# ueda0319/neddf

Measured on AMD Instinct MI355X. Metric: rendered rays/sec (800x800, 128 samples/ray), higher is better.
Workload: dtype f32

## Files before the change

### neddf_amd/csrc/tile_engine.h

```cpp
#pragma once
#include "kernels.h"
#include "device_math.h"

namespace neddf {

typedef float f32x16 __attribute__((ext_vector_type(16)));
typedef float f32x4v __attribute__((ext_vector_type(4)));
typedef __bf16 bf16x8 __attribute__((ext_vector_type(8)));
typedef unsigned short u16x4 __attribute__((ext_vector_type(4)));
typedef unsigned int u32x4 __attribute__((ext_vector_type(4)));

#ifdef NEDDF_EXACT_ACT
#define NEDDF_ACT_F32 0
#define NEDDF_ACT_SPLIT 0
#endif
#ifndef NEDDF_ACT_F32
#define NEDDF_ACT_F32 2
#endif
#ifndef NEDDF_ACT_SPLIT
#define NEDDF_ACT_SPLIT 2
#endif

template <int WID>
struct OpsF32T {
    static constexpr int kWid = WID;
    typedef float act_t;
    typedef f32x4v frag;
    typedef frag afrag;
    typedef frag bfrag;
    static constexpr int kLd = WID + 4;
    static constexpr int kStep = 8;
    static constexpr int kSub = 4;
    static constexpr bool kFast = false;
    static constexpr int kActMode = NEDDF_ACT_F32;
    static constexpr int kPlanes = 1, kPlane = 0;
    static constexpr bool kPackedRows = false;
    static constexpr float kWScale = 1.0f;
    static constexpr bool kStash16 = false;
    static constexpr bool kDeepPrefetch = false;
    static constexpr bool kEncInLds = false;
    static constexpr bool kTransposed = false, kStashF16 = false;
    typedef frag mfrag;
    static __device__ __forceinline__ frag load_a(const act_t *p) { return *(const frag *)p; }
    static __device__ __forceinline__ const mfrag &prep(const frag &a) { return a; }
    static __device__ __forceinline__ void zero(act_t *p) { *p = 0.f; }
    static __device__ __forceinline__ void put4(act_t *p, const f32x4v &v) { *(f32x4v *)p = v; }
    static __device__ __forceinline__ void put(act_t *p, float v) { *p = v; }
    static __device__ __forceinline__ void put2(act_t *pa, act_t *pb, float va, float vb) { *pa = va; *pb = vb; }
    static __device__ __forceinline__ float get(const act_t *p) { return *p; }
    static __device__ __forceinline__ void load4(const act_t *p, float (&x)[4])
    {
        f32x4v v = *(const f32x4v *)p;
        x[0] = v[0]; x[1] = v[1]; x[2] = v[2]; x[3] = v[3];
    }
    static __device__ __forceinline__ f32x16 mfma(const frag &a, const frag &b, const f32x16 &c, int r)
    {
        return __builtin_amdgcn_mfma_f32_32x32x2f32(a[r], b[r], c, 0, 0, 0);
    }
};

typedef OpsF32T<256> OpsF32;

template <int WID>
struct OpsBF16T {
    static constexpr int kWid = WID;
    typedef unsigned short act_t;
    typedef bf16x8 frag;
    typedef frag afrag;
    typedef frag bfrag;
    static constexpr int kLd = WID + 8;
    static constexpr int kStep = 16;
    static constexpr int kSub = 1;
    static constexpr bool kFast = true;
    static constexpr int kActMode = 1;
    static constexpr int kPlanes = 1, kPlane = 0;
    static constexpr float kWScale = 1.0f;
    static constexpr bool kStash16 = true;
    static constexpr bool kDeepPrefetch = true;
    static constexpr bool kEncInLds = true;
    static constexpr bool kTransposed = false, kStashF16 = false;
    typedef frag mfrag;
    static __device__ __forceinline__ frag load_a(const act_t *p) { return *(const frag *)p; }
    static __device__ __forceinline__ const mfrag &prep(const frag &a) { return a; }
    static __device__ __forceinline__ void zero(act_t *p) { *p = 0; }
    static __device__ __forceinline__ unsigned short cvt(float v)
    {
        typedef __bf16 bf16x2 __attribute__((ext_vector_type(2)));
        typedef float f32x2 __attribute__((ext_vector_type(2)));
        f32x2 in = { v, v };
        bf16x2 o = __builtin_convertvector(in, bf16x2);
        return __builtin_bit_cast(unsigned int, o) & 0xffffu;
    }
    static __device__ __forceinline__ void put(act_t *p, float v) { *p = cvt(v); }
    static __device__ __forceinline__ void put2(act_t *pa, act_t *pb, float va, float vb)
    {
        typedef __bf16 bf16x2 __attribute__((ext_vector_type(2)));
        typedef float f32x2 __attribute__((ext_vector_type(2)));
        const unsigned int w = __builtin_bit_cast(unsigned int, __builtin_convertvector((f32x2){ va, vb }, bf16x2));
        *pa = (unsigned short)w; *pb = (unsigned short)(w >> 16);
    }
    static constexpr bool kPackedRows = true;
    static __device__ __forceinline__ void put_rows4(act_t *p, int ld, float v0, float v1, float v2, float v3)
    {
        typedef __bf16 bf16x2 __attribute__((ext_vector_type(2)));
        typedef float f32x2 __attribute__((ext_vector_type(2)));
        const unsigned int a = __builtin_bit_cast(unsigned int, __builtin_convertvector((f32x2){ v0, v1 }, bf16x2));
        const unsigned int b = __builtin_bit_cast(unsigned int, __builtin_convertvector((f32x2){ v2, v3 }, bf16x2));
        p[0] = (unsigned short)a; p[ld] = (unsigned short)(a >> 16);
        p[2 * ld] = (unsigned short)b; p[3 * ld] = (unsigned short)(b >> 16);
    }
    static __device__ __forceinline__ float get(const act_t *p) { return __builtin_bit_cast(float, (unsigned int)*p << 16); }
    static __device__ __forceinline__ void load4(const act_t *p, float (&x)[4])
    {
        u16x4 v = *(const u16x4 *)p;
#pragma unroll
        for (int i = 0; i < 4; ++i) x[i] = __builtin_bit_cast(float, (unsigned int)v[i] << 16);
    }
    static __device__ __forceinline__ f32x16 mfma(const frag &a, const frag &b, const f32x16 &c, int)
    {
        return __builtin_amdgcn_mfma_f32_32x32x16_bf16(a, b, c, 0, 0, 0);
    }
};
typedef OpsBF16T<256> OpsBF16;

template <int WID>
struct OpsBF16RT : OpsBF16T<WID> {
    typedef OpsBF16T<WID> Base;
    typedef typename Base::act_t act_t;
    typedef typename Base::frag frag;
    static constexpr bool kTransposed = true, kStashF16 = true;
    static __device__ __forceinline__ f32x16 mfma(const frag &a, const frag &b, const f32x16 &c, int)
    {
        return __builtin_amdgcn_mfma_f32_32x32x16_bf16(b, a, c, 0, 0, 0);
    }
    static __device__ __forceinline__ void put4(act_t *p, float v0, float v1, float v2, float v3)
    {
        typedef __bf16 bf16x2 __attribute__((ext_vector_type(2)));
        typedef float f32x2 __attribute__((ext_vector_type(2)));
        typedef unsigned int u32x2 __attribute__((ext_vector_type(2)));
        u32x2 w = { __builtin_bit_cast(unsigned int, __builtin_convertvector((f32x2){ v0, v1 }, bf16x2)),
                    __builtin_bit_cast(unsigned int, __builtin_convertvector((f32x2){ v2, v3 }, bf16x2)) };
        *(u32x2 *)p = w;
    }
};

typedef _Float16 f16x8 __attribute__((ext_vector_type(8)));
struct hfrag2 {
    f16x8 h, m;
};

template <int WID>
struct OpsF16SplitT {
    static constexpr int kWid = WID;
    typedef unsigned short act_t;
    typedef hfrag2 afrag;
    typedef hfrag2 bfrag;
    static constexpr int kPlanes = 2, kPlane = WID + 8;
    static constexpr int kLd = 2 * (WID + 8) + 8;
    static constexpr int kStep = 16;
    static constexpr int kSub = 3;
    static constexpr bool kFast = false;
    static constexpr int kActMode = NEDDF_ACT_SPLIT;
    static constexpr bool kPackedRows = false;
    static constexpr float kWScale = 1024.0f;
    static constexpr bool kStash16 = false;
    static constexpr bool kDeepPrefetch = false;
    static constexpr bool kEncInLds = false;
    static constexpr bool kTransposed = false, kStashF16 = false;
    static __device__ __forceinline__ float f(unsigned short b) { return (float)__builtin_bit_cast(_Float16, b); }
    static __device__ __forceinline__ void put(act_t *p, float v)
    {
        typedef __fp16 h2 __attribute__((ext_vector_type(2)));
        h2 t = __builtin_amdgcn_cvt_pkrtz(v, v);
        const _Float16 h = (_Float16)t[0];
        const _Float16 m = (_Float16)__builtin_amdgcn_fmed3f(v - (float)h, -65504.0f, 65504.0f);
        p[0] = __builtin_bit_cast(unsigned short, h);
        p[kPlane] = __builtin_bit_cast(unsigned short, m);
    }
    static __device__ __forceinline__ void put2(act_t *pa, act_t *pb, float va, float vb) { put(pa, va); put(pb, vb); }
    static __device__ __forceinline__ void zero(act_t *p) { p[0] = 0; p[kPlane] = 0; }
    static __device__ __forceinline__ void put4(act_t *p, const f32x4v &v)
    {
        typedef __fp16 h2 __attribute__((ext_vector_type(2)));
        typedef _Float16 f16x4 __attribute__((ext_vector_type(4)));
        f16x4 h, m;
#pragma unroll
        for (int i = 0; i < 4; ++i) {
            h2 t = __builtin_amdgcn_cvt_pkrtz(v[i], v[i]);
            h[i] = (_Float16)t[0];
            m[i] = (_Float16)__builtin_amdgcn_fmed3f(v[i] - (float)h[i], -65504.0f, 65504.0f);
        }
        *(f16x4 *)p = h;
        *(f16x4 *)(p + kPlane) = m;
    }
    static __device__ __forceinline__ float get(const act_t *p) { return f(p[kPlane]) + f(p[0]); }
    static __device__ __forceinline__ void load4(const act_t *p, float (&x)[4])
    {
        u16x4 h = *(const u16x4 *)p, m = *(const u16x4 *)(p + kPlane);
#pragma unroll
        for (int i = 0; i < 4; ++i) x[i] = f(m[i]) + f(h[i]);
    }
    static __device__ __forceinline__ afrag load_a(const act_t *p)
    {
        afrag a;
        a.h = *(const f16x8 *)p; a.m = *(const f16x8 *)(p + kPlane);
        return a;
    }
    typedef afrag mfrag;
    static __device__ __forceinline__ const mfrag &prep(const afrag &a) { return a; }
    static __device__ __forceinline__ f32x16 mfma(const afrag &a, const bfrag &b, const f32x16 &c, int r)
    {
        switch (r) {
        case 0: return __builtin_amdgcn_mfma_f32_32x32x16_f16(a.m, b.h, c, 0, 0, 0);
        case 1: return __builtin_amdgcn_mfma_f32_32x32x16_f16(a.h, b.m, c, 0, 0, 0);
        default: return __builtin_amdgcn_mfma_f32_32x32x16_f16(a.h, b.h, c, 0, 0, 0);
        }
    }
};
typedef OpsF16SplitT<256> OpsF16Split;

struct f32x8frag {
    f32x4v lo, hi;
};
struct bf16x8x3 {
    bf16x8 t[3];
};

template <int WID>
struct OpsF32x3T : OpsF32T<WID> {
    typedef float act_t;
    typedef f32x8frag afrag;
    typedef bf16x8x3 bfrag;
    typedef bf16x8x3 mfrag;
    static constexpr int kStep = 16;
    static constexpr int kSub = 6;
    static __device__ __forceinline__ afrag load_a(const act_t *p) { return { *(const f32x4v *)p, *(const f32x4v *)(p + 4) }; }
    static __device__ __forceinline__ unsigned cvt2(float x0, float x1, float &y0, float &y1)
    {
        typedef __bf16 bf16x2 __attribute__((ext_vector_type(2)));
        typedef float f32x2 __attribute__((ext_vector_type(2)));
        unsigned w = __builtin_bit_cast(unsigned, __builtin_convertvector((f32x2){ x0, x1 }, bf16x2));
        asm("" : "+v"(w));
        y0 = __builtin_bit_cast(float, w << 16);
        y1 = __builtin_bit_cast(float, w & 0xffff0000u);
        return w;
    }
    static __device__ __forceinline__ mfrag prep(const afrag &a)
    {
        const float x[8] = { a.lo[0], a.lo[1], a.lo[2], a.lo[3], a.hi[0], a.hi[1], a.hi[2], a.hi[3] };
        u32x4 t0, t1, t2;
#pragma unroll
        for (int i = 0; i < 4; ++i) {
            float h0, h1, m0, m1, d0, d1;
            t0[i] = cvt2(x[2 * i], x[2 * i + 1], h0, h1);
            const float r0 = x[2 * i] - h0, r1 = x[2 * i + 1] - h1;
            t1[i] = cvt2(r0, r1, m0, m1);
            t2[i] = cvt2(r0 - m0, r1 - m1, d0, d1);
            (void)d0; (void)d1;
        }
        mfrag m;
        m.t[0] = __builtin_bit_cast(bf16x8, t0); m.t[1] = __builtin_bit_cast(bf16x8, t1); m.t[2] = __builtin_bit_cast(bf16x8, t2);
        return m;
    }
    static __device__ __forceinline__ f32x16 mfma(const mfrag &a, const bfrag &b, const f32x16 &c, int r)
    {
        switch (r) {
        case 0: return __builtin_amdgcn_mfma_f32_32x32x16_bf16(a.t[2], b.t[0], c, 0, 0, 0);
        case 1: return __builtin_amdgcn_mfma_f32_32x32x16_bf16(a.t[1], b.t[1], c, 0, 0, 0);
        case 2: return __builtin_amdgcn_mfma_f32_32x32x16_bf16(a.t[0], b.t[2], c, 0, 0, 0);
        case 3: return __builtin_amdgcn_mfma_f32_32x32x16_bf16(a.t[1], b.t[0], c, 0, 0, 0);
        case 4: return __builtin_amdgcn_mfma_f32_32x32x16_bf16(a.t[0], b.t[1], c, 0, 0, 0);
        default: return __builtin_amdgcn_mfma_f32_32x32x16_bf16(a.t[0], b.t[0], c, 0, 0, 0);
        }
    }
};

constexpr int kEncLd = 72;
template <class Ops>
struct EncView : Ops {
    static constexpr int kLd = kEncLd;
};

template <class Ops>
__device__ __forceinline__ const typename Ops::act_t *act_lane_ptr(const typename Ops::act_t *act, int lane)
{
    return act + (lane & 31) * Ops::kLd + (Ops::kStep / 2) * (lane >> 5);
}

struct WeightStream {
    __amdgpu_buffer_rsrc_t rsrc;
    unsigned lane_off;
};

template <class F>
__device__ __forceinline__ WeightStream weight_stream(const F *wl)
{
    const unsigned lane = __builtin_amdgcn_mbcnt_hi(~0u, __builtin_amdgcn_mbcnt_lo(~0u, 0u));
    const unsigned long long u = (unsigned long long)(wl - lane);
    const unsigned lo = __builtin_amdgcn_readfirstlane((unsigned)u), hi = __builtin_amdgcn_readfirstlane((unsigned)(u >> 32));
    void *base = (void *)(((unsigned long long)hi << 32) | lo);
    return { __builtin_amdgcn_make_buffer_rsrc(base, 0, (int)0xffffffffu, 0x00020000), lane * (unsigned)sizeof(F) };
}

template <class F>
__device__ __forceinline__ F stream_load(const WeightStream &w, unsigned frag_index)
{
    static_assert(sizeof(F) % 16 == 0, "fragments are fetched 16 bytes at a time");
    struct Raw { u32x4 v[sizeof(F) / 16]; } raw;
#pragma unroll
    for (unsigned i = 0; i < sizeof(F) / 16; ++i)
        raw.v[i] = __builtin_amdgcn_raw_buffer_load_b128(w.rsrc, w.lane_off + 16 * i, frag_index * (64 * (unsigned)sizeof(F)), 0);
    return __builtin_bit_cast(F, raw);
}

template <int MT, int NT, class Ops = OpsF32>
__device__ __forceinline__ void dense_load(typename Ops::afrag (&a)[MT], typename Ops::bfrag (&b)[NT], const typename Ops::act_t *ap,
                                           const WeightStream &w, int ksteps, int S)
{
#pragma unroll
    for (int t = 0; t < NT; ++t) b[t] = stream_load<typename Ops::bfrag>(w, (unsigned)(t * ksteps + S));
#pragma unroll
    for (int mt = 0; mt < MT; ++mt) a[mt] = Ops::load_a(ap + mt * 32 * Ops::kLd);
}

template <int MT, int NT, class Ops = OpsF32>
__device__ __forceinline__ void dense_mfma(f32x16 (&acc)[MT][NT], const typename Ops::afrag (&a)[MT], const typename Ops::bfrag (&b)[NT])
{
    typename Ops::mfrag m[MT];
#pragma unroll
    for (int mt = 0; mt < MT; ++mt) m[mt] = Ops::prep(a[mt]);
#pragma unroll
    for (int r = 0; r < Ops::kSub; ++r)
#pragma unroll
        for (int mt = 0; mt < MT; ++mt)
#pragma unroll
            for (int t = 0; t < NT; ++t) acc[mt][t] = Ops::mfma(m[mt], b[t], acc[mt][t], r);
}

template <int NT, class Ops = OpsF32>
struct LayerPre {
    typename Ops::bfrag b[NT];
    float bias[NT];
};

template <int NT, class Ops = OpsF32>
__device__ __forceinline__ void layer_prefetch(LayerPre<NT, Ops> &p, const void *wp, const float *bias, int ksteps, int wave, int lane)
{
    const typename Ops::bfrag *wl = (const typename Ops::bfrag *)wp + (size_t)wave * NT * ksteps * 64 + lane;
#pragma unroll
    for (int t = 0; t < NT; ++t) {
        p.b[t] = wl[(size_t)t * ksteps * 64];
        p.bias[t] = bias ? Ops::kWScale * bias[(wave * NT + t) * 32 + (lane & 31)] : 0.f;
    }
    __builtin_amdgcn_sched_barrier(0);
}

template <int MT, int NT, bool ROWS4, class Ops = OpsF32>
__device__ __forceinline__ void acc_init_pre(f32x16 (&acc)[MT][NT], const LayerPre<NT, Ops> &p)
{
#pragma unroll
    for (int t = 0; t < NT; ++t)
#pragma unroll
        for (int mt = 0; mt < MT; ++mt)
#pragma unroll
            for (int q = 0; q < 16; ++q) acc[mt][t][q] = (ROWS4 && (q & 3)) ? 0.f : p.bias[t];
}

#ifndef NEDDF_PROBE_NOB
#define NEDDF_PROBE_NOB 0
#endif
#ifndef NEDDF_PROBE_NOY
#define NEDDF_PROBE_NOY 0
#endif
#ifndef NEDDF_PROBE_NOA
#define NEDDF_PROBE_NOA 0
#endif
template <int MT, int NT, class Ops>
__device__ __forceinline__ void dense_pipeline3(f32x16 (&acc)[MT][NT], typename Ops::afrag (&a0)[MT], typename Ops::bfrag (&b0)[NT],
                                                const typename Ops::act_t *act_lane, const WeightStream &wl, int ksteps)
{

    typename Ops::afrag a[2][MT];
    typename Ops::bfrag b[3][NT];
#pragma unroll
    for (int mt = 0; mt < MT; ++mt) a[0][mt] = a0[mt];
#pragma unroll
    for (int t = 0; t < NT; ++t) {
        b[0][t] = b0[t];
        b[1][t] = stream_load<typename Ops::bfrag>(wl, (unsigned)(t * ksteps + (ksteps > 1 ? 1 : 0)));
    }
    const typename Ops::act_t *ap = act_lane;
    for (int S = 0; S < ksteps; S += 6) {
#pragma unroll
        for (int u = 0; u < 6; ++u) {
            if (S + u >= ksteps) break;
            const int s2 = S + u + 2 < ksteps ? S + u + 2 : ksteps - 1;
#if !NEDDF_PROBE_NOB
#pragma unroll
            for (int t = 0; t < NT; ++t) b[(u + 2) % 3][t] = stream_load<typename Ops::bfrag>(wl, (unsigned)(t * ksteps + s2));
#else
            (void)s2;
#pragma unroll
            for (int t = 0; t < NT; ++t) b[(u + 2) % 3][t] = b[u % 3][t];
#endif
#if !NEDDF_PROBE_NOA
#pragma unroll
            for (int mt = 0; mt < MT; ++mt) a[(u + 1) & 1][mt] = Ops::load_a(ap + (u + 1) * Ops::kStep + mt * 32 * Ops::kLd);
#else
#pragma unroll
            for (int mt = 0; mt < MT; ++mt) a[(u + 1) & 1][mt] = a[u & 1][mt];
#endif
            __builtin_amdgcn_sched_barrier(0);
            dense_mfma<MT, NT, Ops>(acc, a[u & 1], b[u % 3]);
            __builtin_amdgcn_sched_barrier(0);
        }
        ap += 6 * Ops::kStep;
    }
}

template <int MT, int NT, class Ops = OpsF32>
__device__ __forceinline__ void dense_pipeline(f32x16 (&acc)[MT][NT], typename Ops::afrag (&a0)[MT], typename Ops::bfrag (&b0)[NT],
                                               const typename Ops::act_t *act_lane, const WeightStream &wl, int ksteps)
{
    if constexpr (Ops::kDeepPrefetch) {
        dense_pipeline3<MT, NT, Ops>(acc, a0, b0, act_lane, wl, ksteps);
        return;
    }
    typename Ops::afrag a1[MT];
    typename Ops::bfrag b1[NT];
    const typename Ops::act_t *ap = act_lane;
    for (int S = 0; S < ksteps; S += 2) {
        const bool more = S + 1 < ksteps;
        dense_load<MT, NT, Ops>(a1, b1, ap + Ops::kStep, wl, ksteps, more ? S + 1 : S);
        __builtin_amdgcn_sched_barrier(0);
        dense_mfma<MT, NT, Ops>(acc, a0, b0);
        __builtin_amdgcn_sched_barrier(0);
        if (more) {
            dense_load<MT, NT, Ops>(a0, b0, ap + 2 * Ops::kStep, wl, ksteps, S + 2 < ksteps ? S + 2 : S);
            __builtin_amdgcn_sched_barrier(0);
            dense_mfma<MT, NT, Ops>(acc, a1, b1);
            __builtin_amdgcn_sched_barrier(0);
        }
        ap += 2 * Ops::kStep;
    }
}

template <int MT, int NT, class Ops = OpsF32>
__device__ __forceinline__ void dense_pre(f32x16 (&acc)[MT][NT], const typename Ops::act_t *act_lane, const typename Ops::bfrag *wl,
                                          int ksteps, const LayerPre<NT, Ops> &p)
{
    typename Ops::afrag a0[MT];
    typename Ops::bfrag b0[NT];
#pragma unroll
    for (int t = 0; t < NT; ++t) b0[t] = p.b[t];
#pragma unroll
    for (int mt = 0; mt < MT; ++mt) a0[mt] = Ops::load_a(act_lane + mt * 32 * Ops::kLd);
    dense_pipeline<MT, NT, Ops>(acc, a0, b0, act_lane, weight_stream(wl), ksteps);
}

template <int MT, int NT, class Ops = OpsF32>
__device__ __forceinline__ void dense(f32x16 (&acc)[MT][NT], const typename Ops::act_t *act_lane, const typename Ops::bfrag *wl, int ksteps)
{
    typename Ops::afrag a0[MT];
    typename Ops::bfrag b0[NT];
    const WeightStream w = weight_stream(wl);
    dense_load<MT, NT, Ops>(a0, b0, act_lane, w, ksteps, 0);
    dense_pipeline<MT, NT, Ops>(acc, a0, b0, act_lane, w, ksteps);
}

template <int MT, int NT, class Ops = OpsF32>
__device__ __forceinline__ void dense_from_zero(f32x16 (&acc)[MT][NT], const typename Ops::act_t *act_lane, const typename Ops::bfrag *wl, int ksteps)
{
#pragma unroll
    for (int mt = 0; mt < MT; ++mt)
#pragma unroll
        for (int t = 0; t < NT; ++t)
#pragma unroll
            for (int q = 0; q < 16; ++q) acc[mt][t][q] = 0.f;
    dense<MT, NT, Ops>(acc, act_lane, wl, ksteps);
}

template <int MT, int NT, bool ROWS4>
__device__ __forceinline__ void acc_init(f32x16 (&acc)[MT][NT], const float *bias, int wave, int lane, float scale = 1.0f)
{
#pragma unroll
    for (int t = 0; t < NT; ++t) {
        float bv = bias ? scale * bias[(wave * NT + t) * 32 + (lane & 31)] : 0.f;
#pragma unroll
        for (int mt = 0; mt < MT; ++mt)
#pragma unroll
            for (int q = 0; q < 16; ++q) acc[mt][t][q] = (ROWS4 && (q & 3)) ? 0.f : bv;
    }
}

template <int MT, int NT>
__device__ __forceinline__ void stash_store(const f32x16 (&acc)[MT][NT], float *slot, int wave, int lane)
{
    f32x4v *dst = (f32x4v *)slot + (size_t)wave * (MT * NT * 4) * 64 + lane;
#pragma unroll
    for (int mt = 0; mt < MT; ++mt)
#pragma unroll
        for (int t = 0; t < NT; ++t)
#pragma unroll
            for (int g = 0; g < 4; ++g) {
                f32x4v v = { acc[mt][t][4 * g], acc[mt][t][4 * g + 1], acc[mt][t][4 * g + 2], acc[mt][t][4 * g + 3] };
                dst[((mt * NT + t) * 4 + g) * 64] = v;
            }
}

template <int MT, int NT>
__device__ __forceinline__ void stash_store16(const f32x16 (&acc)[MT][NT], float *slot, int wave, int lane)
{
    typedef __bf16 bf16x2 __attribute__((ext_vector_type(2)));
    typedef float f32x2 __attribute__((ext_vector_type(2)));
    u32x4 *dst = (u32x4 *)slot + (size_t)wave * (MT * NT * 2) * 64 + lane;
#pragma unroll
    for (int mt = 0; mt < MT; ++mt)
#pragma unroll
        for (int t = 0; t < NT; ++t)
#pragma unroll
            for (int c = 0; c < 2; ++c) {
                u32x4 v;
#pragma unroll
                for (int i = 0; i < 4; ++i)
                    v[i] = __builtin_bit_cast(unsigned int, __builtin_convertvector((f32x2){ acc[mt][t][8 * c + 2 * i], acc[mt][t][8 * c + 2 * i + 1] }, bf16x2));
                dst[((mt * NT + t) * 2 + c) * 64] = v;
            }
}

__device__ __forceinline__ void stash_load16(f32x16 &dst, const u32x4 *src)
{
#pragma unroll
    for (int c = 0; c < 2; ++c) {
        const u32x4 v = src[c * 64];
#pragma unroll
        for (int i = 0; i < 4; ++i) {
            dst[8 * c + 2 * i] = __builtin_bit_cast(float, v[i] << 16);
            dst[8 * c + 2 * i + 1] = __builtin_bit_cast(float, v[i] & 0xffff0000u);
        }
    }
}

typedef _Float16 f16x2 __attribute__((ext_vector_type(2)));
template <int MT, int NT>
__device__ __forceinline__ void stash_store_f16(const f32x16 (&acc)[MT][NT], float *slot, int wave, int lane)
{
    typedef float f32x2 __attribute__((ext_vector_type(2)));
    u32x4 *dst = (u32x4 *)slot + (size_t)wave * (MT * NT * 2) * 64 + lane;
#pragma unroll
    for (int mt = 0; mt < MT; ++mt)
#pragma unroll
        for (int t = 0; t < NT; ++t)
#pragma unroll
            for (int c = 0; c < 2; ++c) {
                u32x4 v;
#pragma unroll
                for (int i = 0; i < 4; ++i)
                    v[i] = __builtin_bit_cast(unsigned int, __builtin_convertvector((f32x2){ acc[mt][t][8 * c + 2 * i], acc[mt][t][8 * c + 2 * i + 1] }, f16x2));
                dst[((mt * NT + t) * 2 + c) * 64] = v;
            }
}

template <int HI>
__device__ __forceinline__ float mul_f16_half(unsigned w, float x)
{
    float d;
    if constexpr (HI) asm("v_fma_mix_f32 %0, %1, %2, 0 op_sel:[1,0,0] op_sel_hi:[1,0,0]" : "=v"(d) : "v"(w), "v"(x));
    else asm("v_fma_mix_f32 %0, %1, %2, 0 op_sel:[0,0,0] op_sel_hi:[1,0,0]" : "=v"(d) : "v"(w), "v"(x));
    return d;
}

template <int MT, int NT>
__device__ __forceinline__ void stash_add(f32x16 (&acc)[MT][NT], const float *slot, int wave, int lane)
{
    const f32x4v *src = (const f32x4v *)slot + (size_t)wave * (MT * NT * 4) * 64 + lane;
#pragma unroll
    for (int mt = 0; mt < MT; ++mt)
#pragma unroll
        for (int t = 0; t < NT; ++t)
#pragma unroll
            for (int g = 0; g < 4; ++g) {
                f32x4v v = src[((mt * NT + t) * 4 + g) * 64];
                acc[mt][t][4 * g] += v[0]; acc[mt][t][4 * g + 1] += v[1];
                acc[mt][t][4 * g + 2] += v[2]; acc[mt][t][4 * g + 3] += v[3];
            }
}

template <int MT, int NT, bool ROWS4, int KIND, class Ops = OpsF32>
__device__ __forceinline__ void epilogue(const f32x16 (&acc)[MT][NT], typename Ops::act_t *act, int wave, int lane)
{
    constexpr int LD = Ops::kLd;
    const int j = lane & 31, h = lane >> 5;
#pragma unroll
    for (int mt = 0; mt < MT; ++mt)
#pragma unroll
        for (int t = 0; t < NT; ++t) {
            typename Ops::act_t *o = act + (mt * 32 + 4 * h) * LD + (wave * NT + t) * 32 + j;
#pragma unroll
            for (int g = 0; g < 4; ++g) {
                float z[4];
#pragma unroll
                for (int r = 0; r < 4; ++r) {
                    z[r] = acc[mt][t][4 * g + r];
                    if constexpr (Ops::kWScale != 1.0f) z[r] *= (1.0f / Ops::kWScale);
                }
                if constexpr (Ops::kPackedRows) {
                    typedef float f32x2 __attribute__((ext_vector_type(2)));
                    if (ROWS4) {
                        f32x2 lo, hi;
                        if constexpr (KIND == 2 && Ops::kActMode == 1) {
                            float tx, dy;
                            tanhexp_parts_fast(z[0], tx, dy);
                            lo = (f32x2){ z[0] * tx, z[1] * dy };
                            hi = (f32x2){ z[2] * dy, z[3] * dy };
                        } else {
                            float y, dy;
                            act_grad<KIND, Ops::kActMode>(z[0], y, dy);
                            lo = (f32x2){ y, dy * z[1] };
                            hi = (f32x2){ z[2] * dy, z[3] * dy };
                        }
                        Ops::put_rows4(o + (8 * g) * LD, LD, lo[0], lo[1], hi[0], hi[1]);
                    } else {
                        Ops::put_rows4(o + (8 * g) * LD, LD, act_val<KIND, Ops::kActMode>(z[0]), act_val<KIND, Ops::kActMode>(z[1]),
                                       act_val<KIND, Ops::kActMode>(z[2]), act_val<KIND, Ops::kActMode>(z[3]));
                    }
                } else if (ROWS4) {
                    float y, dy;
                    act_grad<KIND, Ops::kActMode>(z[0], y, dy);
                    Ops::put2(o + (8 * g + 0) * LD, o + (8 * g + 1) * LD, y, dy * z[1]);
                    Ops::put2(o + (8 * g + 2) * LD, o + (8 * g + 3) * LD, dy * z[2], dy * z[3]);
                } else {
#pragma unroll
                    for (int r = 0; r < 4; r += 2)
                        Ops::put2(o + (8 * g + r) * LD, o + (8 * g + r + 1) * LD, act_val<KIND, Ops::kActMode>(z[r]), act_val<KIND, Ops::kActMode>(z[r + 1]));
                }
            }
        }
}

template <int MT, int NT, bool ROWS4, class Ops = OpsF32>
__device__ __forceinline__ void epilogue_rt(const f32x16 (&acc)[MT][NT], typename Ops::act_t *act, int kind, int wave, int lane)
{
    if (kind == 0) epilogue<MT, NT, ROWS4, 0, Ops>(acc, act, wave, lane);
    else if (kind == 1) epilogue<MT, NT, ROWS4, 1, Ops>(acc, act, wave, lane);
    else epilogue<MT, NT, ROWS4, 2, Ops>(acc, act, wave, lane);
}

template <class Ops = OpsF32, int THREADS = kThreads>
__device__ __forceinline__ void zero_cols(typename Ops::act_t *act, int rows, int ncols, int tid)
{
    typedef typename Ops::act_t act_t;
    constexpr int E = 16 / (int)sizeof(act_t);
    if (ncols % E == 0 && (Ops::kLd * (int)sizeof(act_t)) % 16 == 0 && (Ops::kPlane * (int)sizeof(act_t)) % 16 == 0) {
        const int cpr = ncols / E;
        for (int i = tid; i < rows * cpr; i += THREADS) {
            const int r = i / cpr, c = i - r * cpr;
#pragma unroll
            for (int pl = 0; pl < Ops::kPlanes; ++pl) *(f32x4v *)(act + r * Ops::kLd + pl * Ops::kPlane + c * E) = (f32x4v){ 0.f, 0.f, 0.f, 0.f };
        }
        return;
    }
    for (int i = tid; i < rows * ncols; i += THREADS) {
        int r = i / ncols, c = i - r * ncols;
        Ops::zero(act + r * Ops::kLd + c);
    }
}

}
```

Baseline: 642,900.

## Overlap split-precision A-fragment prep with MFMAs via sched group barriers

For ops types whose A fragment needs a conversion (f32 split into three bf16 parts), the dense pipeline now precomputes the next step's split fragments and runs that work in the same block as the current step's MFMAs. sched_group_barrier calls interleave the conversion VALU instructions between MFMAs so they can hide under matrix latency. The cost is extra live registers for the double-buffered split fragments, which could lower occupancy or cause spills.

Result: faster. 664,000, median of 6 (+3.3%).

```diff
diff --git a/neddf_amd/csrc/tile_engine.h b/neddf_amd/csrc/tile_engine.h
--- a/neddf_amd/csrc/tile_engine.h
+++ b/neddf_amd/csrc/tile_engine.h
@@ -234,6 +234,7 @@
     typedef bf16x8x3 mfrag;
     static constexpr int kStep = 16;
     static constexpr int kSub = 6;
+    static constexpr int kPrepValu = 44;
     static __device__ __forceinline__ afrag load_a(const act_t *p) { return { *(const f32x4v *)p, *(const f32x4v *)(p + 4) }; }
     static __device__ __forceinline__ unsigned cvt2(float x0, float x1, float &y0, float &y1)
     {
@@ -418,12 +419,61 @@
     }
 }
 
+template <class Ops>
+constexpr bool kSplitsA = !std::is_same<typename Ops::afrag, typename Ops::mfrag>::value;
+
+template <int MT, int NT, class Ops>
+__device__ __forceinline__ void dense_mfma_split(f32x16 (&acc)[MT][NT], const typename Ops::mfrag (&m)[MT], const typename Ops::bfrag (&b)[NT],
+                                                 const typename Ops::afrag (&an)[MT], typename Ops::mfrag (&mn)[MT])
+{
+#pragma unroll
+    for (int r = 0; r < Ops::kSub; ++r)
+#pragma unroll
+        for (int mt = 0; mt < MT; ++mt)
+#pragma unroll
+            for (int t = 0; t < NT; ++t) acc[mt][t] = Ops::mfma(m[mt], b[t], acc[mt][t], r);
+#pragma unroll
+    for (int mt = 0; mt < MT; ++mt) mn[mt] = Ops::prep(an[mt]);
+    constexpr int kMfma = Ops::kSub * MT * NT, kLead = MT * NT;
+    constexpr int kPer = (Ops::kPrepValu * MT + kMfma - kLead - 1) / (kMfma - kLead);
+#pragma unroll
+    for (int i = 0; i < kLead; ++i) __builtin_amdgcn_sched_group_barrier(0x008, 1, 0);
+#pragma unroll
+    for (int i = kLead; i < kMfma; ++i) {
+        __builtin_amdgcn_sched_group_barrier(0x008, 1, 0);
+        __builtin_amdgcn_sched_group_barrier(0x002, kPer, 0);
+    }
+}
+
 template <int MT, int NT, class Ops = OpsF32>
 __device__ __forceinline__ void dense_pipeline(f32x16 (&acc)[MT][NT], typename Ops::afrag (&a0)[MT], typename Ops::bfrag (&b0)[NT],
                                                const typename Ops::act_t *act_lane, const WeightStream &wl, int ksteps)
 {
     if constexpr (Ops::kDeepPrefetch) {
         dense_pipeline3<MT, NT, Ops>(acc, a0, b0, act_lane, wl, ksteps);
+        return;
+    }
+    if constexpr (kSplitsA<Ops>) {
+        typename Ops::afrag a1[MT];
+        typename Ops::bfrag b1[NT];
+        typename Ops::mfrag m0[MT], m1[MT];
+#pragma unroll
+        for (int mt = 0; mt < MT; ++mt) m0[mt] = Ops::prep(a0[mt]);
+        const typename Ops::act_t *ap = act_lane;
+        for (int S = 0; S < ksteps; S += 2) {
+            const bool more = S + 1 < ksteps;
+            dense_load<MT, NT, Ops>(a1, b1, ap + Ops::kStep, wl, ksteps, more ? S + 1 : S);
+            __builtin_amdgcn_sched_barrier(0);
+            dense_mfma_split<MT, NT, Ops>(acc, m0, b0, a1, m1);
+            __builtin_amdgcn_sched_barrier(0);
+            if (more) {
+                dense_load<MT, NT, Ops>(a0, b0, ap + 2 * Ops::kStep, wl, ksteps, S + 2 < ksteps ? S + 2 : S);
+                __builtin_amdgcn_sched_barrier(0);
+                dense_mfma_split<MT, NT, Ops>(acc, m1, b1, a0, m0);
+                __builtin_amdgcn_sched_barrier(0);
+            }
+            ap += 2 * Ops::kStep;
+        }
         return;
     }
     typename Ops::afrag a1[MT];
```
